# ShawnHymel/ei-keyword-spotting

Hardware: AMD Instinct MI355X
Metric: 1s@16kHz clips/sec (MFCC+CNN) (higher is better)
Workload: dtype f32

## Files before the change

### ei-keyword-spotting_amd/csrc/kws_device.h

```cpp
#pragma once
#include <hip/hip_runtime.h>
#include <stdint.h>
#include <float.h>
#include <type_traits>

#include "kws_plan.h"
#include "../../include/kws/kws_synth.h"

#pragma clang fp contract(off)

#define KWS_WAVE 64

__device__ __forceinline__ int sel_count(const int *sel, int n_clips) { return sel ? min(sel[0], n_clips) : n_clips; }
__device__ __forceinline__ int sel_clip(const int *sel, int i) { return sel ? sel[1 + i] : i; }

#define WAVE_SYNC()                                                   \
    do {                                                              \
        __builtin_amdgcn_fence(__ATOMIC_RELEASE, "wavefront");        \
        __builtin_amdgcn_wave_barrier();                              \
        __builtin_amdgcn_fence(__ATOMIC_ACQUIRE, "wavefront");        \
    } while (0)

__device__ __forceinline__ int ring_out_row(const KwsDspPlan &P, int r) { return P.ring_rows ? (P.ring_row0 + r) % P.ring_rows : r; }
__device__ __forceinline__ int ring_in_row(const KwsDspPlan &P, int i) { return (P.ring_rows && i < P.ring_rows) ? (i + P.ring_head) % P.ring_rows : i; }
// ... 11 lines not shown
__device__ __forceinline__ cf cadd(cf a, cf b) { cf c; c.r = a.r + b.r; c.i = a.i + b.i; return c; }
__device__ __forceinline__ cf csub(cf a, cf b) { cf c; c.r = a.r - b.r; c.i = a.i - b.i; return c; }

__device__ __forceinline__ void bfly4(cf &f0, cf &f1, cf &f2, cf &f3, cf t1, cf t2, cf t3)
{
    cf s0 = cmul(f1, t1), s1 = cmul(f2, t2), s2 = cmul(f3, t3);
    cf s5 = csub(f0, s1);
    f0 = cadd(f0, s1);
    cf s3 = cadd(s0, s2), s4 = csub(s0, s2);
    f2 = csub(f0, s3);
    f0 = cadd(f0, s3);
    f1.r = s5.r + s4.i;
    f1.i = s5.i - s4.r;
    f3.r = s5.r - s4.i;
    f3.i = s5.i + s4.r;
}

__device__ __forceinline__ void bfly4_unit(cf &f0, cf &f1, cf &f2, cf &f3)
{
    const cf s0 = f1, s1 = f2, s2 = f3;
    cf s5 = csub(f0, s1);
    f0 = cadd(f0, s1);
    cf s3 = cadd(s0, s2), s4 = csub(s0, s2);
    f2 = csub(f0, s3);
    f0 = cadd(f0, s3);
    f1.r = s5.r + s4.i;
    f1.i = s5.i - s4.r;
    f3.r = s5.r - s4.i;
    f3.i = s5.i + s4.r;
}

typedef int fast_i2 __attribute__((ext_vector_type(2), aligned(4)));

__device__ __forceinline__ cf exact_point(fast_i2 v, float pre_cof)
{
    const float prev = (float)(v.x >> 16) * (1.0f / 32768.0f);
    const float lo = (float)(short)(v.y & 0xffff) * (1.0f / 32768.0f);
    const float hi = (float)(v.y >> 16) * (1.0f / 32768.0f);
    cf z;
    const float pl = pre_cof * prev;
    z.r = lo - pl;
    const float ph_ = pre_cof * lo;
    z.i = hi - ph_;
    return z;
}

// ... 164 lines not shown
```

### ei-keyword-spotting_amd/csrc/kws_fast.h

```cpp
#pragma once
#include <stdint.h>

#include "kws_plan.h"

#define KWS_FAST_MAX_BLOCKS 8
#define KWS_FAST_NZ_MAX 12
#define KWS_FAST_NZ2 8
#define KWS_FAST_DCT_GROUPS 5
#define KWS_FAST_MEL_CHUNK 8
#define KWS_FAST_CMVN_EXT 8
#define KWS_FAST_XS 144
#define KWS_FAST_WAVE 64
#ifndef KWS_FAST_WPS
#define KWS_FAST_WPS 2
#endif
#define KWS_FAST_ZF 320

struct KwsFastBlock {
    int in_w, in_c, in_cp;
    int out_c, taps, pad_left, out_w;
    int pool, pool_stride, pool_w;
    int in_stride;
    int m_tiles, n_tiles;
    int vrows;
// ... 35 lines not shown
    int guard_off;
    int guard_cep_off;
    float v_net_feat;
    float g_c1, g_c2, v_net, lvl_inv;
    float c0_factor, c0_abs, c0_rel, c0_inv_rows;
    int pad_off;
    int sil_off;
    float sys_t2;
    int fs, f_floats, r1_floats, wave_floats, shared_floats, n_waves;
    int zero_off;
    int sink_off;
    int stash_off;
    const float *shared_init;
    int qnet, q_floats;
    int mfe;
    int fuse, n_blocks;
    KwsFastBlock blk[KWS_FAST_MAX_BLOCKS];
    int fc_in, fc_out, fc_w_off, fc_b_off;
    float fc_min, fc_max, beta;
    int n_labels;
    int wps;
    int twl_off;
    int *tickets;
};
```

### ei-keyword-spotting_amd/csrc/kws_fast.hip

```cpp
#include <atomic>

#include "kws_device.h"
#include "kws_fast.h"
#if KWS_FAST_WPS >= 3
#define kws_fast_kernel kws_fast_kernel_w3
#define kws_launch_fast kws_launch_fast_w3
#define kws_launch_fast_prof kws_launch_fast_prof_w3
#endif
#include "kws_nn_int8_dev.h"

typedef float v4f __attribute__((ext_vector_type(4)));
#if KWS_FAST_WPS >= 3
#define KWS_OPAQUE3(v) asm volatile("" : "+v"(v))
#define KWS_FAST_SINK (shared + FP.sink_off)
#else
#define KWS_OPAQUE3(v) do { } while (0)
#define KWS_FAST_SINK (F + FP.sink_off)
#endif
static_assert(KWS_FAST_ZF == KWS_ZF && KWS_FAST_WAVE == KWS_WAVE, "kws_fast.h mirrors kws_device.h");

template <int CTRL> __device__ __forceinline__ float dpp_mov(float v)
{
    return __int_as_float(__builtin_amdgcn_update_dpp(0, __float_as_int(v), CTRL, 0xf, 0xf, true));
}
// ... 222 lines not shown
        __builtin_amdgcn_sched_barrier(0);
        if (it + 1 >= n_it) break;
        const int tap1 = d1.y;
        d1 = steps[it + 3];
        fetch(d2, a0, b0);
        d0 = d2;
        __builtin_amdgcn_sched_barrier(0);
        clip_rows(tap1, a1);
        mfmas(a1, b1);
        __builtin_amdgcn_sched_barrier(0);
    }
    __builtin_amdgcn_s_setprio(0);
    if (t_loop) *t_loop = clock64();
    fast_conv_finish<MT, NT>(k, acc, vout, stage, sstride, shared, lane, sink, 1.0f);
    return 1.0f;
}

typedef _Float16 v8h __attribute__((ext_vector_type(8)));
typedef _Float16 v2h __attribute__((ext_vector_type(2)));
typedef const __attribute__((address_space(1))) char *kws_gptr;
typedef const __attribute__((address_space(1))) v8h *kws_gv8h;
#define KWS_FAST_HP 16

template <int T>
__device__ __forceinline__ float fast_split_trips(float *__restrict__ img, int items, int in_c, int in_cp, int in_stride, int lane, unsigned inv, int ppr)
{
    float2 v[T];
    int off[T];
    int pc[T];
#pragma unroll
    for (int u = 0; u < T; ++u) {
        const int i = min(lane + KWS_WAVE * u, items - 1);
        const int r = (int)(__umul24((unsigned)i, inv) >> 20), p2 = 2 * (i - __mul24(r, ppr));
        const int ro = __mul24(r, in_stride);
        v[u] = *(const float2 *)(img + ro + p2);
        off[u] = 4 * ro + 2 * p2;
        pc[u] = p2;
    }
#pragma unroll
    for (int u = 0; u < T; ++u) asm volatile("" : "+v"(v[u].x), "+v"(v[u].y));
    float mx = 0.0f;
#pragma unroll
    for (int u = 0; u < T; ++u) {
        v[u].x = pc[u] < in_c ? v[u].x : 0.0f;
        v[u].y = pc[u] + 1 < in_c ? v[u].y : 0.0f;
        mx = fmaxf(mx, fmaxf(fabsf(v[u].x), fabsf(v[u].y)));
    }
    mx = wave_max(mx);
    const int e = __builtin_amdgcn_readfirstlane(min(max(__builtin_amdgcn_frexp_expf(mx), -100), 100));
    const float s = ldexpf(1.0f, 14 - e);
    WAVE_SYNC();
    char *const ib = (char *)img;
    const int lo_off = 2 * in_cp;
#pragma unroll
    for (int u = 0; u < T; ++u) {
        const float y0 = v[u].x * s, y1 = v[u].y * s;
        const _Float16 h0 = (_Float16)y0, h1 = (_Float16)y1;
        const float d0 = y0 - (float)h0, d1 = y1 - (float)h1;
        const v2h hi = { h0, h1 }, lo = { (_Float16)d0, (_Float16)d1 };
        *(v2h *)(ib + off[u]) = hi;
        *(v2h *)(ib + off[u] + lo_off) = lo;
    }
    WAVE_SYNC();
    return ldexpf(1.0f, e - 14);
}

__device__ __forceinline__ float fast_split_image(float *__restrict__ img, int in_w, int in_c, int in_cp, int in_stride, int lane, unsigned ppr_inv20)
{
    const int ppr = in_cp >> 1, items = in_w * ppr;
    if (items <= 4 * KWS_WAVE) return fast_split_trips<4>(img, items, in_c, in_cp, in_stride, lane, ppr_inv20, ppr);
    if (items <= 8 * KWS_WAVE) return fast_split_trips<8>(img, items, in_c, in_cp, in_stride, lane, ppr_inv20, ppr);
    return fast_split_trips<KWS_FAST_HP>(img, items, in_c, in_cp, in_stride, lane, ppr_inv20, ppr);
}

template <int MT>
__device__ __forceinline__ float fast_conv_small_h(const KwsFastBlock &k, float *__restrict__ in, float *__restrict__ stage, int sstride,
                                                   const float *__restrict__ shared, int zero_off, int lane, float *__restrict__ sink)
{
    constexpr int KSM = 8;
    const int lm = lane & 15, lq = lane >> 4, n_ks = k.h_ks;
    const kws_gptr bg = (kws_gptr)k.h_b_global + lane * 16;
    v8h bh[KSM], blo[KSM];
#pragma unroll
    for (int ks = 0; ks < KSM; ++ks) {
        const int kc = min(ks, n_ks - 1);
        bh[ks] = *(kws_gv8h)(bg + (kc * 2) * (KWS_WAVE * 16));
        blo[ks] = *(kws_gv8h)(bg + (kc * 2 + 1) * (KWS_WAVE * 16));
    }
    const float inv_s = fast_split_image(in, k.in_w, k.in_c, k.in_cp, k.in_stride, lane, k.inv_ppr20);
    v4f acc[MT][1];
#pragma unroll
    for (int mt = 0; mt < MT; ++mt) acc[mt][0] = v4f{ 0.f, 0.f, 0.f, 0.f };
    const int rowb = k.in_stride * 4, in_w = k.in_w, lo_off = 2 * k.in_cp;
    const int row0 = lm - k.pad_left;
    const char *const abase = (const char *)in + row0 * rowb;
// ... 484 lines not shown
    if constexpr (QCP != 0) {
        unsigned char *const qs = (unsigned char *)(lds + FP.shared_floats);
        const KwsNnPlan &QN = *QNp;
        for (int i = threadIdx.x * 4; i < QN.blk[0].out_c * 256; i += blockDim.x * 4) *(int *)(qs + i) = *(const int *)(QN.blk[0].add_lut + i);
        for (int i = threadIdx.x * 4; i < QN.blk[1].out_c * 256; i += blockDim.x * 4) *(int *)(qs + 32 * 256 + i) = *(const int *)(QN.blk[1].add_lut + i);
        (void)nn_head_stage(QN, qs + Q_HEAD);
        nn_mfma_stage_lds<QCP == 0 ? 16 : QCP>(QN, (v4i *)(qs + Q_WB1), (v4i *)(qs + Q_WB2), (int *)(qs + Q_RQ));
    }
    if constexpr (FROM_CEP)
        for (int i = lane; i < FP.wave_floats; i += KWS_WAVE) F[i] = 0.0f;
    __syncthreads();

    const int nfr = P.n_frames, ncep = P.n_cepstral, NF = 8 * DG;
    const int n_tail = (nfr >= KWS_FAST_MEL_CHUNK && (nfr & 7) != 0 && (nfr & 7) <= 2) ? (nfr & 7) : 0;
    const int n_pass = n_tail ? nfr / KWS_FAST_MEL_CHUNK : (nfr + KWS_FAST_MEL_CHUNK - 1) / KWS_FAST_MEL_CHUNK;
    const int fs = FP.fs;
    float *img = F;
    float *elog = F + nfr * fs;
    constexpr int NZ2 = DG > 4 ? KWS_FAST_NZ2 : 1;
    const float *dct_frag = shared + FP.dct_off;
    const int pstride = FP.pstride;
    const int n_waves = blockDim.x >> 6;
    const float pre_cof = P.pre_cof, pscale = P.inv_fft * (1.0f / 1073741824.0f) * 0.25f;
    const int frame_stride = P.frame_stride, n_samples = P.n_samples;
    const float *cnt_tab = shared + FP.cnt_off;
    const int *upd_tab = (const int *)(shared + FP.upd_off);
    const float *ext_tab = FP.ext_off >= 0 ? shared + FP.ext_off : nullptr;
    const float inv_win = FP.inv_win;
    const float *guard_tab = shared + (FROM_CEP ? FP.guard_cep_off : FP.guard_off);
    const int *pad_idx = (const int *)(shared + FP.pad_off);
    const int win_size = P.win_size, prow = nfr + 2 * P.pad;
    const int cr = FP.cr, n_blocks = FP.n_blocks, n_labels = FP.n_labels;
    long long ph[KWS_FAST_NPHASE] = { 0 }, tlast = PROF ? clock64() : 0;

    const int clip_stride = gridDim.x * n_waves;
    float *const stash = F + FP.stash_off;
    bool have_stash = false;
    const int n_sel = FROM_CEP ? sel_count(sel, n_clips) : n_clips;
#if KWS_FAST_WPS >= 3
    int *const tk = FP.tickets;
    int tv = 0;
    int ni = 0;
    auto draw = [&]() { if (ni < n_sel && lane == 0) tv = __hip_atomic_fetch_add(tk, 1, __ATOMIC_RELAXED, __HIP_MEMORY_SCOPE_AGENT); };
    draw();
    ni = clip_stride + __builtin_amdgcn_readfirstlane(tv);
    draw();
    for (int ci = blockIdx.x * n_waves + wave; ci < n_sel; ci = ni, ni = ni < n_sel ? clip_stride + __builtin_amdgcn_readfirstlane(tv) : ni, draw()) {
        const int clip = FROM_CEP ? sel_clip(sel, ci) : ci;
        const int next_ci = ni;
        const int next_clip = ni < n_sel ? ni : -1;
#else
    for (int ci = blockIdx.x * n_waves + wave; ci < n_sel; ci += clip_stride) {
        const int clip = FROM_CEP ? sel_clip(sel, ci) : ci;
        const int next_ci = ci + clip_stride;
        const int next_clip = ci + clip_stride < n_sel ? ci + clip_stride : -1;
#endif
        int lane_c = lane;
        asm volatile("" : "+v"(lane_c));
        const int fl = lane_c & 7, fg = lane_c >> 3;
        const int nbA = (fl >> 2) + 4 * (fl & 3);
        const cf a1 = to_cf(P.tw[16]), a2 = to_cf(P.tw[32]), a3 = to_cf(P.tw[48]);
        const cf b1 = to_cf(P.tw[4 * fl]), b2 = to_cf(P.tw[8 * fl]), b3 = to_cf(P.tw[12 * fl]);
#if KWS_FAST_WPS >= 3
        const float *const twl_c = shared + FP.twl_off + 24 * fl, *const twl_s = shared + FP.twl_off + 192 + 16 * fl;
#else
        cf c1[4], c2[4], c3[4];
    #pragma unroll
        for (int a = 0; a < 4; ++a) { c1[a] = to_cf(P.tw[fl + 8 * a]); c2[a] = to_cf(P.tw[2 * (fl + 8 * a)]); c3[a] = to_cf(P.tw[3 * (fl + 8 * a)]); }
        cf stw[8];
    #pragma unroll
        for (int q = 0; q < 8; ++q) {
            const int k = fl + 8 * (q & 3) + 32 * (q >> 2);
            stw[q] = to_cf(P.stw[(k == 0 ? KWS_NC / 2 : k) - 1]);
        }
#endif
        const int xwr = fg * KWS_FAST_XS + 18 * fl;
        const int xrd = fg * KWS_FAST_XS + 2 * fl;
        const int partner = (lane_c & ~7) | ((8 - fl) & 7);
        const int half = lane_c >> 5, t = lane_c & 31;
        const int start1 = FP.tap_start1[lane_c], start2 = FP.tap_start2[lane_c];
        float lvl_sum = 0.0f;
        float w1[NZ], w2[NZ2];
    #pragma unroll
        for (int n = 0; n < NZ; ++n) w1[n] = FP.tap_w1[lane_c * KWS_FAST_NZ_MAX + n];
// ... 59 lines not shown
                if (s2 >= 2 * pairs) break;
                float xv[2][NZ];
#pragma unroll
                for (int s = 0; s < 2; ++s)
#pragma unroll
                    for (int n = 0; n < NZ; ++n) xv[s][n] = p1[(s2 + s) * pstride + n];
#pragma unroll
                for (int s = 0; s < 2; ++s) {
                    float acc = 0.0f;
#pragma unroll
                    for (int n = 0; n < NZ; ++n) acc = __fmaf_rn(xv[s][n], w1[n], acc);
                    macc[s2 + s] = acc;
                }
            }
            float acc2 = 0.0f;
            if (DG > 4) {
                float xv2[NZ2];
#pragma unroll
                for (int n = 0; n < NZ2; ++n) xv2[n] = p2[n];
#pragma unroll
                for (int n = 0; n < NZ2; ++n) acc2 = __fmaf_rn(xv2[n], w2[n], acc2);
            }
            macc[4] = acc2;
#pragma unroll
            for (int s = 0; s < 5; ++s) {
                const float a = macc[s] == 0.0f ? FLT_EPSILON : macc[s];
                macc[s] = MFE ? a : fast_log(a);
            }
#pragma unroll
            for (int s = 0; s < 4; ++s) {
                const int slot = 4 * half + s;
                if (slot < nfc && t < NF) img[(fbase + slot) * fs + t + (slot == 1 ? adj1 : 0)] = macc[s];
            }
            if (DG > 4 && sl2 < nfc && j2 < NF) img[(fbase + sl2) * fs + j2 + (sl2 == 1 ? adj1 : 0)] = macc[4];
        };
        fast_i2 nxt[2][8];
        fetch(0, nxt);
        int touched = touch(1);
        const bool pair_tail = n_tail == 1 && !have_stash && next_clip >= 0;
        int touched_tail = 0;
        const int16_t *const xnext = pcm + (size_t)max(next_clip, 0) * n_samples;
        if (pair_tail && lane_c < 8) touched_tail = *(const int *)(xnext + (nfr - 1) * frame_stride + 32 * lane_c);
        for (int q = 0; q < n_pass; ++q) {
            const int fbase = KWS_FAST_MEL_CHUNK * q;
            const int f = fbase + fg;
            const bool live = f < nfr;
            cf u[4][4];
            {
                cf z[2][8];
#pragma unroll
                for (int blk = 0; blk < 2; ++blk)
#pragma unroll
                    for (int i = 0; i < 8; ++i) z[blk][i] = fast_point(nxt[blk][i], pre_cof);
                if (f == 0 && fl == 0) {
                    fast_i2 v = nxt[0][0];
                    v.y = v.x;
                    v.x = wrap_prev << 16;
                    z[0][0] = fast_point(v, pre_cof);
                }
                fetch(q + 1, nxt);
                asm volatile("" : : "v"(touched));
                touched = touch(q + 2);
                FPH(0);
#pragma unroll
                for (int blk = 0; blk < 2; ++blk) {
                    cf sm[4], df[4];
#pragma unroll
                    for (int i = 0; i < 4; ++i) { sm[i] = cadd(z[blk][2 * i], z[blk][2 * i + 1]); df[i] = csub(z[blk][2 * i], z[blk][2 * i + 1]); }
                    bfly4_unit(sm[0], sm[1], sm[2], sm[3]);
                    bfly4(df[0], df[1], df[2], df[3], a1, a2, a3);
#pragma unroll
                    for (int i = 0; i < 4; ++i) { z[blk][2 * i] = sm[i]; z[blk][2 * i + 1] = df[i]; }
                }
#pragma unroll
                for (int rnd = 0; rnd < 2; ++rnd) {
#pragma unroll
                    for (int r = 0; r < 8; ++r) *(float2 *)(xw + xwr + 2 * r) = make_float2(z[rnd][r].r, z[rnd][r].i);
                    WAVE_SYNC();
#pragma unroll
                    for (int b = 0; b < 2; ++b)
#pragma unroll
                        for (int a = 0; a < 4; ++a) {
                            const float2 v = *(const float2 *)(xw + xrd + 18 * a + 72 * b);
                            u[a][2 * rnd + b].r = v.x; u[a][2 * rnd + b].i = v.y;
                        }
                    WAVE_SYNC();
                }
            }
#pragma unroll
            for (int b = 0; b < 4; ++b) bfly4(u[0][b], u[1][b], u[2][b], u[3][b], b1, b2, b3);
#pragma unroll
#if KWS_FAST_WPS >= 3
            for (int a = 0; a < 4; ++a) {
// ... 19 lines not shown
                float esum = 0.0f;
#pragma unroll
                for (int qq = 0; qq < 8; ++qq) {
                    const int a = qq & 3, b = qq >> 2;
                    cf other;
                    other.r = __int_as_float(__builtin_amdgcn_ds_bpermute(partner << 2, __float_as_int(u[3 - a][3 - b].r)));
                    other.i = __int_as_float(__builtin_amdgcn_ds_bpermute(partner << 2, __float_as_int(u[3 - a][3 - b].i)));
                    cf fpk = u[a][b];
                    int k = fl + 8 * a + 32 * b;
                    {
                        const int o = qq == 0 ? 8 : 16 - qq;
                        other.r = lane0 ? u[o & 3][o >> 2].r : other.r;
                        other.i = lane0 ? u[o & 3][o >> 2].i : other.i;
                        if (qq == 0) { fpk.r = lane0 ? u[0][2].r : fpk.r; fpk.i = lane0 ? u[0][2].i : fpk.i; k = lane0 ? KWS_NC / 2 : k; }
                    }
                    cf fpnk; fpnk.r = other.r; fpnk.i = -other.i;
                    const cf f1k = cadd(fpk, fpnk), f2k = csub(fpk, fpnk);
                    const cf twv = cmul(f2k, stw[qq]);
                    cf lo, hi;
                    lo.r = f1k.r + twv.r;
                    lo.i = f1k.i + twv.i;
                    hi.r = f1k.r - twv.r;
                    hi.i = twv.i - f1k.i;
                    const float plo = __fmaf_rn(lo.r, lo.r, lo.i * lo.i) * pscale;
                    const float phi = __fmaf_rn(hi.r, hi.r, hi.i * hi.i) * pscale;
                    prow[k] = plo;
                    esum += (qq == 0 && lane0) ? 0.0f : plo;
                    esum += phi;
                    prow[KWS_NC - k] = phi;
                }
                if (fl == 0) {
                    const float dc = u[0][0].r + u[0][0].i, ny = u[0][0].r - u[0][0].i;
#if KWS_FAST_WPS >= 3
                    const float pdc = ((dc * dc) * pscale) * 4.0f, pny = ((ny * ny) * pscale) * 4.0f;
#else
                    const float pdc = (dc * dc) * (4.0f * pscale), pny = (ny * ny) * (4.0f * pscale);
#endif
                    esum += pdc + pny;
                    prow[0] = pdc;
                }
                esum = oct_sum(esum);
                if (fl == 0 && live) elog[f] = fast_log(esum == 0.0f ? FLT_EPSILON : esum);
            }
            FPH(2);

            mel_phase(fbase, min(KWS_FAST_MEL_CHUNK, nfr - fbase), 2, 0);
            WAVE_SYNC();
            FPH(3);
        }

        asm volatile("" : : "v"(touched_tail));
        if (n_tail == 1 && have_stash) {
            if (lane_c < NF) img[(nfr - 1) * fs + lane_c] = stash[lane_c];
            if (lane_c == 47) elog[nfr - 1] = stash[47];
            have_stash = false;
            WAVE_SYNC();
        } else if (n_tail) {
            const int16_t *const xb_t = (pair_tail && half == 1) ? xnext : xbase;
            const int ft = pair_tail ? nfr - 1 : KWS_FAST_MEL_CHUNK * n_pass + half;
            const bool live_t = ft < nfr;
            const int s0 = min(ft, nfr - 1) * frame_stride + 8 * t;
            const int4 rawv = *(const int4 *)(xb_t + s0);
            const int rawp = s0 == 0 ? wrap_prev : (int)xb_t[s0 - 1];
            const int k01 = t & 1, g01 = t >> 1, n0 = (g01 >> 2) + 4 * (g01 & 3), K2 = t & 7, G2 = t >> 3;
// ... 47 lines not shown
                const cf st1 = to_cf(P.stw[t]), st2 = to_cf(P.stw[t + 32]);
                cf fpk[2], fq[2];
#pragma unroll
                for (int rep = 0; rep < 2; ++rep) {
                    const int k = t + 1 + 32 * rep;
                    fpk[rep] = ld_cf(zb, k);
                    fq[rep] = ld_cf(zb, KWS_NC - k);
                }
                const float2 d0 = *(const float2 *)zb;
                float *prow = pw + half * pstride;
                float esum = 0.0f;
#pragma unroll
                for (int rep = 0; rep < 2; ++rep) {
                    const int k = t + 1 + 32 * rep;
                    const cf stw_ = rep ? st2 : st1;
                    cf fpnk; fpnk.r = fq[rep].r; fpnk.i = -fq[rep].i;
                    const cf f1k = cadd(fpk[rep], fpnk), f2k = csub(fpk[rep], fpnk);
                    const cf twv = cmul(f2k, stw_);
                    cf lo, hi;
                    lo.r = f1k.r + twv.r;
                    lo.i = f1k.i + twv.i;
                    hi.r = f1k.r - twv.r;
                    hi.i = twv.i - f1k.i;
                    const float plo = __fmaf_rn(lo.r, lo.r, lo.i * lo.i) * pscale;
                    const float phi = __fmaf_rn(hi.r, hi.r, hi.i * hi.i) * pscale;
                    if (k != KWS_NC / 2) {
                        esum += plo;
                        prow[k] = plo;
                    }
                    esum += phi;
                    prow[KWS_NC - k] = phi;
                }
                if (t == 0) {
                    const float dc = d0.x + d0.y, ny = d0.x - d0.y;
                    const float pdc = (dc * dc) * (4.0f * pscale), pny = (ny * ny) * (4.0f * pscale);
                    esum += pdc + pny;
                    prow[0] = pdc;
                }
                esum = half_wave_sum(esum);
                if (t == 0 && live_t) *((pair_tail && half == 1) ? stash + 47 : elog + ft) = fast_log(esum == 0.0f ? FLT_EPSILON : esum);
            }
            mel_phase(KWS_FAST_MEL_CHUNK * n_pass, pair_tail ? 2 : n_tail, 1, pair_tail ? (int)(stash - img) - nfr * fs : 0);
            have_stash = pair_tail;
            WAVE_SYNC();
        }

        if constexpr (!MFE) {
            int lane_l = lane;
            asm volatile("" : "+v"(lane_l));
            const int lm = lane_l & 15, lq = lane_l >> 4;
            float dB[DG][2][2];
#pragma unroll
            for (int g = 0; g < DG; ++g)
#pragma unroll
                for (int i = 0; i < 2; ++i)
#pragma unroll
                    for (int nt = 0; nt < 2; ++nt) dB[g][i][nt] = dct_frag[((g * 2 + i) * 2 + nt) * KWS_WAVE + lane_l];
            const float *arow = img + lm * fs + 2 * lq;
            float e0 = 0.0f;
            if (lane_l < nfr) e0 = elog[lane_l];
            v4f acc[4][2];
            __builtin_amdgcn_s_setprio(1);
// ... 405 lines not shown
```

### ei-keyword-spotting_amd/csrc/kws_fast_plan.cpp

```cpp
#include "kws_internal.h"
#include <atomic>
#include <cstdlib>

static const int kLdsBytes = 160 * 1024;

static int round_up(int v, int m) { return (v + m - 1) / m * m; }

static uint16_t f32_to_f16(float f)
{
    uint32_t u;
    memcpy(&u, &f, sizeof u);
    const uint32_t sign = (u >> 16) & 0x8000u;
    u &= 0x7fffffffu;
    if (u >= 0x47800000u) return (uint16_t)(sign | (u > 0x7f800000u ? 0x7e00u : 0x7c00u));
    if (u < 0x38800000u) {
        if (u < 0x33000000u) return (uint16_t)sign;
        const int shift = 126 - (int)(u >> 23);
        const uint32_t m = (u & 0x7fffffu) | 0x800000u;
        uint32_t h = m >> shift;
        const uint32_t rem = m & ((1u << shift) - 1u), half = 1u << (shift - 1);
        if (rem > half || (rem == half && (h & 1u))) h++;
        return (uint16_t)(sign | h);
    }
    uint32_t h = ((u - 0x38000000u) >> 13);
// ... 32 lines not shown
{
    h->fast_sil_row.clear();
    if (h->model.dsp.block == DSP_BLOCK_MFE || h->dsp.generic) return;
    const int nfr = h->dsp.n_frames, ncep = h->dsp.n_cepstral;
    const size_t ns = (size_t)h->dsp.n_samples, nv = (size_t)nfr * (size_t)ncep;
    int16_t *d_pcm = nullptr;
    float *d_cep = nullptr;
    std::vector<float> cep(nv, 0.0f);
    bool ok = hipMalloc((void **)&d_pcm, ns * sizeof(int16_t) + 64) == hipSuccess && hipMalloc((void **)&d_cep, nv * sizeof(float)) == hipSuccess;
    ok = ok && hipMemset(d_pcm, 0, ns * sizeof(int16_t) + 64) == hipSuccess && hipMemset(d_cep, 0xff, nv * sizeof(float)) == hipSuccess;
    ok = ok && spectral_device(h, h->dsp, d_pcm, 0, 1, d_cep, nullptr, nullptr) == EI_IMPULSE_OK && hipDeviceSynchronize() == hipSuccess;
    ok = ok && hipMemcpy(cep.data(), d_cep, nv * sizeof(float), hipMemcpyDeviceToHost) == hipSuccess;
    if (d_pcm) (void)hipFree(d_pcm);
    if (d_cep) (void)hipFree(d_cep);
    (void)hipGetLastError();
    if (!ok) return;
    for (int c = 0; c < ncep; c++) {
        if (!std::isfinite(cep[(size_t)c])) return;
        for (int r = 1; r < nfr; r++)
            if (memcmp(&cep[(size_t)r * ncep + c], &cep[(size_t)c], sizeof(float)) != 0) return;
    }
    if (fabsf(cep[0] - logf(FLT_EPSILON)) > 1.0e-3f) return;
    h->fast_sil_row.assign(cep.begin(), cep.begin() + ncep);
}

static void build_guard(kws_handle *h, KwsFastPlan &F, std::vector<float> &shared)
{
    const int ncep = h->dsp.n_cepstral, NF = h->model.dsp.num_filters, nfr = h->dsp.n_frames;
    const bool refit = h->is_float && h->gain.calibrated;
    float a0 = refit ? kAlpha0 : 1.0e-7f, ad = refit ? -1.0f : kAlphaDct, as = refit ? kAlphaStale : 4.0e-8f, kappa = refit ? kKappa : 0.5e-6f, scale = 1.0f;
    const float e0 = refit ? kAbs0 : 6.0e-7f, kappa_s = refit ? kKappaStale : 0.35e-6f, kappa_0 = refit ? kKappa0 : 0.5e-6f;
    if (const char *ev = KWS_DEV_ENV("KWS_DEV_FAST_GUARD_SCALE")) { scale = (float)atof(ev); h->fast_dev_overrides |= 1; }
    if (const char *ev = KWS_DEV_ENV("KWS_DEV_FAST_GUARD")) { (void)sscanf(ev, "%f,%f,%f,%f", &a0, &ad, &as, &kappa); h->fast_dev_overrides |= 2; }
    if (KWS_DEV_ENV("KWS_DEV_FAST_NO_RERUN")) h->fast_dev_overrides |= 4;
#ifdef KWS_DEV_SWITCHES
    if (h->fast_dev_overrides) {
        static std::atomic<bool> said{ false };
        if (!said.exchange(true))
            fprintf(stderr, "libkws_mi355x: a KWS_DEV_FAST_* development switch is set: KWS_MODE_FAST results are OUTSIDE the documented tolerance\n");
    }
#endif
    std::vector<float> gain((size_t)ncep, 0.0f);
    if (h->is_float && h->gain.calibrated) gain = h->gain.col;
    else for (float &g : gain) g = 4.0f / (kGuardLin * sqrtf((float)(nfr * ncep)));
    h->fast_gain_used = gain;
    F.g_c1 = (kGuardK * kGuardLin / kGuardScoreTol) * (kGuardK * kGuardLin / kGuardScoreTol);
// ... 24 lines not shown
                coef[1] = 0.0f;
                coef[2] = g * kap;
                coef[3] = c == 0 ? 0.0f : g * kKappaSilent;
            }
            for (int k = 0; k < 4; k++) {
                shared.push_back(coef[k]);
                if (c < ncep) h->fast_guard_coef[tier][k].push_back(k == 1 ? coef[k] * unit : coef[k]);
            }
        }
    }
    {
        int entry = 3;
        for (int tier = 1; tier >= 0; tier--) {
            double v = (double)F.v_net;
            for (int c = 0; c < ncep; c++) {
                const double dev = c == 0 ? 1.5 : c <= NF / 2 ? 1.0 : 0.5, mean = c == 0 ? 8.0 : c <= NF / 2 ? 1.0 : 2.2;
                const double b = ((double)h->fast_guard_coef[tier][0][(size_t)c] + (double)h->fast_guard_coef[tier][1][(size_t)c] * 10.0 +
                                  (double)h->fast_guard_coef[tier][2][(size_t)c] * mean) / dev;
                v += (double)nfr * b * b;
            }
            if (v * (double)std::max(F.g_c1 / 16.0f, F.g_c2) <= 1.0) entry = tier + 1;
        }
        if (const char *ev = KWS_DEV_ENV("KWS_DEV_FAST_ENTRY")) entry = std::max(1, std::min(3, atoi(ev)));
        h->fast_entry_tier = entry;
    }
    std::vector<int> pmap;
    h_pad_map(h->dsp.n_frames, h->dsp.pad, pmap);
    {
        const int nfr = h->dsp.n_frames, win = h->model.dsp.win_size;
        int mult = win;
        for (int r = 0; r < nfr; r++) {
            std::vector<int> cnt((size_t)nfr, 0);
            for (int p = r; p < r + win; p++) cnt[(size_t)pmap[(size_t)p]]++;
            for (int v : cnt) mult = std::min(mult, v);
        }
        F.c0_factor = sqrtf((float)mult * (float)nfr / (float)win) * 0.98f;
        const float budget = 1.0f / std::max(F.g_c1 / 16.0f, F.g_c2);
        const float per_dev = gain[0] * sqrtf((float)nfr / (kC0Share * budget));
        F.c0_abs = scale * kFloorCep * per_dev;
        F.c0_rel = scale * std::min(kappa, kappa_0) * per_dev;
        F.c0_inv_rows = 1.0f / (float)nfr;
    }
    F.sys_t2 = (h->is_float && h->gain.calibrated) ? kSysRatio * kSysRatio : 0.0f;
    F.pad_off = (int)shared.size();
    for (int v : pmap) { float f; memcpy(&f, &v, sizeof f); shared.push_back(f); }
    F.sil_off = -1;
    if ((int)h->fast_sil_row.size() == ncep && !KWS_DEV_ENV("KWS_DEV_FAST_NO_SILENT_ROW")) {
        while (shared.size() & 3) shared.push_back(0.0f);
        F.sil_off = (int)shared.size();
        for (int c = 0; c < 32; c++) shared.push_back((c >= 1 && c <= NF / 2 && c < ncep) ? h->fast_sil_row[(size_t)c] : 0.0f);
    }
}

static EI_IMPULSE_ERROR build_fast_dsp(kws_handle *h, KwsFastPlan &F, std::vector<float> &shared)
{
    const Model &m = h->model;
    const DspCfg &c = m.dsp;
    const KwsDspPlan &P = h->dsp;
    const int NF = c.num_filters, nfr = P.n_frames, ncep = P.n_cepstral;
    F.mfe = c.block == DSP_BLOCK_MFE ? 1 : 0;
    if (P.generic) return fail(KWS_ERROR_UNSUPPORTED_MODEL, "fast mode serves the configurations of the tuned MFCC kernel (fft 256, 32 / 40 filters, "
                                                            "up to 52 aligned frames); this model runs on the general kernels");
    if (c.fft_length != 256) return fail(KWS_ERROR_UNSUPPORTED_MODEL, "fast mode: fft_length %d (kernel is built for 256)", c.fft_length);
    if (NF != 32 && NF != 40) return fail(KWS_ERROR_UNSUPPORTED_MODEL, "fast mode: %d mel filters (the kernel is instantiated for 32 and 40)", NF);
    if ((ncep <= 16 || F.wps >= 3) && nfr <= 52) { F.cr = 13; F.cg = 16; }
    else if (nfr <= 51) { F.cr = 17; F.cg = 20; }
    else return fail(KWS_ERROR_UNSUPPORTED_MODEL, "fast mode: %d frames x %d cepstra outside the cmvnw layouts", nfr, ncep);
    if (nfr < 2) return fail(KWS_ERROR_UNSUPPORTED_MODEL, "fast mode: %d frames", nfr);

    const uint32_t fs_hz = m.frequency;
    const uint32_t high = c.high_frequency == 0 ? fs_hz / 2 : (uint32_t)c.high_frequency;
    const std::vector<float> fb = h_filterbank(NF, P.n_bins, fs_hz, (uint32_t)c.low_frequency, high, c.quantize_fb != 0);
    int bmin = P.n_bins, bmax = -1, max_nz = 0;
    std::vector<std::vector<std::pair<int, float>>> taps(NF);
    for (int j = 0; j < NF; j++) {
        for (int k = 0; k < P.n_bins; k++) {
            const float w = fb[(size_t)k * NF + j];
            if (w != 0.0f) { taps[j].push_back({ k, w }); bmin = std::min(bmin, k); bmax = std::max(bmax, k); }
        }
        max_nz = std::max(max_nz, (int)taps[j].size());
    }
    if (bmax < 0) { bmin = 0; bmax = 0; }
    if (max_nz > KWS_FAST_NZ_MAX) return fail(KWS_ERROR_UNSUPPORTED_MODEL, "fast mode: mel filter with %d taps (at most %d)", max_nz, KWS_FAST_NZ_MAX);
    if (bmax > P.n_bins - 2) return fail(KWS_ERROR_UNSUPPORTED_MODEL, "fast mode: a mel filter reads the Nyquist bin");
    bmin = 0;
    bmax = P.n_bins - 2;
// ... 5 lines not shown
        for (size_t n = 1; n < taps[j].size(); n++)
            if (taps[j][n].first != taps[j][n - 1].first + 1) return fail(KWS_ERROR_UNSUPPORTED_MODEL, "fast mode: mel filter %d has a gap", j);
        (j < 32 ? nz1 : nz2) = std::max(j < 32 ? nz1 : nz2, (int)taps[j].size());
    }
    if (nz1 > KWS_FAST_NZ_MAX || nz2 > KWS_FAST_NZ2)
        return fail(KWS_ERROR_UNSUPPORTED_MODEL, "fast mode: mel filters with %d / %d taps (at most %d / %d)", nz1, nz2, KWS_FAST_NZ_MAX, KWS_FAST_NZ2);
    F.nz = nz1 <= 4 ? 4 : nz1 <= 8 ? 8 : KWS_FAST_NZ_MAX;
    F.pstride = (F.nbins + std::max(F.nz, KWS_FAST_NZ2)) | 1;
    if (F.pstride <= 136) F.pstride = 136;
    auto tap_table = [&](auto filter_of_lane, int width, std::vector<int> &start, std::vector<float> &w) {
        start.assign(KWS_FAST_WAVE, 0);
        w.assign((size_t)KWS_FAST_WAVE * width, 0.0f);
        for (int lane = 0; lane < KWS_FAST_WAVE; lane++) {
            const int j = filter_of_lane(lane);
            if (j < 0 || j >= NF || taps[j].empty()) continue;
            start[lane] = taps[j][0].first - bmin;
            for (size_t n = 0; n < taps[j].size(); n++) w[(size_t)lane * width + n] = taps[j][n].second;
        }
    };
    std::vector<int> s1, s2;
    std::vector<float> tw1, tw2;
    tap_table([&](int lane) { return lane & 31; }, KWS_FAST_NZ_MAX, s1, tw1);
    tap_table([&](int lane) { return F.nf2p ? 32 + (lane & (F.nf2p - 1)) : -1; }, KWS_FAST_NZ2, s2, tw2);

    F.dct_groups = NF / 8;
    F.dct_nt = (NF / 2 + 1 + 15) / 16;
    if (F.dct_nt > 2) return fail(KWS_ERROR_UNSUPPORTED_MODEL, "fast mode: DCT output tiles");
    F.dct_nt = 2;
    F.stale_scale = P.dct_s1;
    std::vector<float> frag((size_t)F.dct_groups * 2 * F.dct_nt * KWS_FAST_WAVE, 0.0f);
    for (int g = 0; g < F.dct_groups; g++)
        for (int i = 0; i < 2; i++)
            for (int nt = 0; nt < F.dct_nt; nt++)
                for (int lane = 0; lane < KWS_FAST_WAVE; lane++) {
                    const int k = 8 * g + 2 * (lane >> 4) + i, n = 16 * nt + (lane & 15);
                    double v = 0.0;
                    if (n <= NF / 2) v = 2.0 * cos(M_PI * (double)n * (double)(2 * k + 1) / (double)(2 * NF)) * (double)(n == 0 ? P.dct_s0 : P.dct_s1);
                    frag[(((size_t)g * 2 + i) * F.dct_nt + nt) * KWS_FAST_WAVE + lane] = (float)v;
                }

    std::vector<int> pmap;
    h_pad_map(nfr, P.pad, pmap);
    const int ng = KWS_FAST_WAVE / F.cg, win = c.win_size;
    F.inv_win = 1.0f / (float)win;
    build_guard(h, F, shared);
    while (shared.size() & 3) shared.push_back(0.0f);
// ... 339 lines not shown
```

### ei-keyword-spotting_amd/csrc/kws_internal.h

```cpp
#pragma once
#include <hip/hip_runtime.h>

#include <float.h>
#include <math.h>
#include <stdarg.h>
#include <stdio.h>
#include <stdlib.h>
#include <string.h>
#include <time.h>

#include <mutex>
#include <string>
#include <map>
#include <vector>

#include "../../include/kws/kws.h"
#include "kws_plan.h"
#include "kws_fast.h"

int kws_launch_spectral(const KwsDspPlan &P, const void *pcm, int pcm_is_float, int n_clips, float *mfcc_out, const float *wrap,
                        int out_stride, int grid_cap, hipStream_t stream, const int *sel = nullptr);
int kws_launch_maf(float *scores, float *running_sum, float *maf_buf, int n, int buf_idx, int taps, hipStream_t stream);
int kws_launch_unring(const float *src, float *dst, int n_streams, int rows, int cols, int ring_rows, int head, hipStream_t stream);
int kws_launch_mfe(const KwsDspPlan &P, const void *pcm, int pcm_is_float, int n_clips, float *mel_out, float *energy_out, const float *wrap,
// ... 77 lines not shown
enum { DSP_BLOCK_MFCC = 0, DSP_BLOCK_MFE = 1 };
struct DspCfg {
    int axes, num_cepstral, num_filters, fft_length, win_size, low_frequency, high_frequency, pre_shift;
    float frame_length, frame_stride, pre_cof;
    int block = DSP_BLOCK_MFCC;
    int quantize_fb = 0;
};
struct Model {
    std::vector<Tensor> t;
    std::vector<Node> n;
    std::vector<std::string> labels;
    uint32_t t_in = 0, t_out = 0, raw_sample_count = 0, frequency = 0, nn_input_frame_size = 0;
    DspCfg dsp;
};

bool parse_model(const void *blob, size_t nbytes, Model &m);
float h_fast_log(float a);
float h_freq_to_mel(float f);
float h_mel_to_freq(float mel);
void h_linspace(float start, float stop, uint32_t number, float *out);
std::vector<float> h_filterbank(int num_filter, int coefficients, uint32_t fs, uint32_t low, uint32_t high, bool quantize = false);
float h_quantize_zero_one(float value);
void h_twiddles(int nfft, std::vector<float2> &tw);
void h_super_twiddles(int ncfft, std::vector<float2> &st);
void h_pad_map(int rows, int pad, std::vector<int> &map);
int32_t h_srdhm(int32_t a, int32_t b);
int32_t h_rdivpot(int32_t x, int e);
void h_quantize_multiplier(double m, int32_t *q, int *shift);
int32_t h_wadd(int32_t a, int32_t b);
int32_t h_wsub(int32_t a, int32_t b);
int32_t h_sat_shl(int32_t x, int e);
int32_t h_exp_interval(int32_t a);
int32_t h_exp_neg_q5_26(int32_t a);
void h_act_range(int activation, float scale, int32_t zp, int32_t *amin, int32_t *amax);
int h_out_size(int padding, int image, int filter, int stride, int dil);
int h_pad_amount(int stride, int dil, int in_size, int filter, int out);

struct kws_handle {
    Model model;
    int device = 0;
    int n_cu = 256;
    KwsDspPlan dsp{};
    KwsNnPlan nn{};
    bool is_float = false;
    KwsNnPlanF32 nnf{};
    const KwsNnPlanF32 *d_nnf = nullptr;
// ... 156 lines not shown
```

Baseline: 52.61 million.

## Fold power scale into mel weights, specialize radix-4 twiddles, streamline split-image addressing

Specializes one radix-4 butterfly for the fixed twiddles (c,-c),(0,-1),(-c,-c), so it needs fewer multiplies. It moves the per-bin power scale out of the per-bin loops: the scale is folded into the mel filter weights when that is exact, or applied to the mel accumulators otherwise, and to the energy after the reduction. The fp16 split of the image now walks LDS addresses incrementally with explicit LDS pointers, and skips the padding masks when channels are not padded. Host checks confirm the twiddle pattern and that the fold is exact, so rounding stays bit-compatible, at the cost of extra plan complexity.

```diff
diff --git a/ei-keyword-spotting_amd/csrc/kws_device.h b/ei-keyword-spotting_amd/csrc/kws_device.h
--- a/ei-keyword-spotting_amd/csrc/kws_device.h
+++ b/ei-keyword-spotting_amd/csrc/kws_device.h
@@ -57,6 +57,31 @@
     cf s5 = csub(f0, s1);
     f0 = cadd(f0, s1);
     cf s3 = cadd(s0, s2), s4 = csub(s0, s2);
+    f2 = csub(f0, s3);
+    f0 = cadd(f0, s3);
+    f1.r = s5.r + s4.i;
+    f1.i = s5.i - s4.r;
+    f3.r = s5.r - s4.i;
+    f3.i = s5.i + s4.r;
+}
+
+__device__ __forceinline__ void bfly4_k1(cf &f0, cf &f1, cf &f2, cf &f3, float c, float e)
+{
+    const float p1 = f1.r * c, q1 = f1.i * c, p3 = f3.r * c, q3 = f3.i * c;
+    const float er = f2.r * e, ei = f2.i * e;
+    cf s0, s1;
+    s0.r = p1 + q1;
+    s0.i = q1 - p1;
+    s1.r = er + f2.i;
+    s1.i = ei - f2.r;
+    const float s2r = q3 - p3, n2 = p3 + q3;
+    cf s5 = csub(f0, s1);
+    f0 = cadd(f0, s1);
+    cf s3, s4;
+    s3.r = s0.r + s2r;
+    s3.i = s0.i - n2;
+    s4.r = s0.r - s2r;
+    s4.i = s0.i + n2;
     f2 = csub(f0, s3);
     f0 = cadd(f0, s3);
     f1.r = s5.r + s4.i;
diff --git a/ei-keyword-spotting_amd/csrc/kws_fast.h b/ei-keyword-spotting_amd/csrc/kws_fast.h
--- a/ei-keyword-spotting_amd/csrc/kws_fast.h
+++ b/ei-keyword-spotting_amd/csrc/kws_fast.h
@@ -81,4 +81,5 @@
     int wps;
     int twl_off;
     int *tickets;
+    int pfold;
 };
diff --git a/ei-keyword-spotting_amd/csrc/kws_fast.hip b/ei-keyword-spotting_amd/csrc/kws_fast.hip
--- a/ei-keyword-spotting_amd/csrc/kws_fast.hip
+++ b/ei-keyword-spotting_amd/csrc/kws_fast.hip
@@ -268,35 +268,54 @@
 typedef const __attribute__((address_space(1))) v8h *kws_gv8h;
 #define KWS_FAST_HP 16
 
-template <int T>
-__device__ __forceinline__ float fast_split_trips(float *__restrict__ img, int items, int in_c, int in_cp, int in_stride, int lane, unsigned inv, int ppr)
+typedef __attribute__((address_space(3))) char *kws_lptr;
+typedef float v2f __attribute__((ext_vector_type(2)));
+template <int T, bool PAD>
+__device__ __forceinline__ float fast_split_trips(float *__restrict__ img, int in_w, int in_c, int in_cp, int in_stride, int lane, unsigned inv, int ppr)
 {
     float2 v[T];
     int off[T];
-    int pc[T];
+    int pc[PAD ? T : 1];
+    constexpr int CLAMP_FROM = T > 4 ? T / 2 : 0;
+    const int base = (int)(unsigned)(uintptr_t)(kws_lptr)(char *)img;
+    const int rowb = 4 * in_stride, rowh = 4 * ppr;
+    const int qr = (int)(__umul24((unsigned)KWS_WAVE, inv) >> 20), qp = KWS_WAVE - __mul24(qr, ppr);
+    const int d_hb = 4 * qp, d_ra = __mul24(qr, rowb) + 2 * d_hb, carry_ra = rowb - 2 * rowh;
+    const int ra_last = base + __mul24(in_w - 1, rowb) + 2 * rowh - 8, off_last = ra_last - (rowh - 4);
+    const int r0 = (int)(__umul24((unsigned)lane, inv) >> 20);
+    int hb = 4 * (lane - __mul24(r0, ppr));
+    int ra = base + __mul24(r0, rowb) + 2 * hb;
 #pragma unroll
     for (int u = 0; u < T; ++u) {
-        const int i = min(lane + KWS_WAVE * u, items - 1);
-        const int r = (int)(__umul24((unsigned)i, inv) >> 20), p2 = 2 * (i - __mul24(r, ppr));
-        const int ro = __mul24(r, in_stride);
-        v[u] = *(const float2 *)(img + ro + p2);
-        off[u] = 4 * ro + 2 * p2;
-        pc[u] = p2;
+        int ru = ra, ou = ra - hb;
+        if (u >= CLAMP_FROM) { ru = min(ru, ra_last); ou = min(ou, off_last); }
+        const v2f rd = *(const __attribute__((address_space(3))) v2f *)(kws_lptr)(uintptr_t)(unsigned)ru;
+        v[u].x = rd.x; v[u].y = rd.y;
+        off[u] = ou;
+        if constexpr (PAD) pc[u] = (ru - ou) >> 1;
+        if (u + 1 < T) {
+            hb += d_hb;
+            ra += d_ra;
+            const bool carry = hb >= rowh;
+            hb = carry ? hb - rowh : hb;
+            ra = carry ? ra + carry_ra : ra;
+        }
     }
 #pragma unroll
     for (int u = 0; u < T; ++u) asm volatile("" : "+v"(v[u].x), "+v"(v[u].y));
     float mx = 0.0f;
 #pragma unroll
     for (int u = 0; u < T; ++u) {
-        v[u].x = pc[u] < in_c ? v[u].x : 0.0f;
-        v[u].y = pc[u] + 1 < in_c ? v[u].y : 0.0f;
+        if constexpr (PAD) {
+            v[u].x = pc[u] < in_c ? v[u].x : 0.0f;
+            v[u].y = pc[u] + 1 < in_c ? v[u].y : 0.0f;
+        }
         mx = fmaxf(mx, fmaxf(fabsf(v[u].x), fabsf(v[u].y)));
     }
     mx = wave_max(mx);
     const int e = __builtin_amdgcn_readfirstlane(min(max(__builtin_amdgcn_frexp_expf(mx), -100), 100));
     const float s = ldexpf(1.0f, 14 - e);
     WAVE_SYNC();
-    char *const ib = (char *)img;
     const int lo_off = 2 * in_cp;
 #pragma unroll
     for (int u = 0; u < T; ++u) {
@@ -304,8 +323,8 @@
         const _Float16 h0 = (_Float16)y0, h1 = (_Float16)y1;
         const float d0 = y0 - (float)h0, d1 = y1 - (float)h1;
         const v2h hi = { h0, h1 }, lo = { (_Float16)d0, (_Float16)d1 };
-        *(v2h *)(ib + off[u]) = hi;
-        *(v2h *)(ib + off[u] + lo_off) = lo;
+        *(__attribute__((address_space(3))) v2h *)(kws_lptr)(uintptr_t)(unsigned)off[u] = hi;
+        *(__attribute__((address_space(3))) v2h *)(kws_lptr)(uintptr_t)(unsigned)(off[u] + lo_off) = lo;
     }
     WAVE_SYNC();
     return ldexpf(1.0f, e - 14);
@@ -314,9 +333,14 @@
 __device__ __forceinline__ float fast_split_image(float *__restrict__ img, int in_w, int in_c, int in_cp, int in_stride, int lane, unsigned ppr_inv20)
 {
     const int ppr = in_cp >> 1, items = in_w * ppr;
-    if (items <= 4 * KWS_WAVE) return fast_split_trips<4>(img, items, in_c, in_cp, in_stride, lane, ppr_inv20, ppr);
-    if (items <= 8 * KWS_WAVE) return fast_split_trips<8>(img, items, in_c, in_cp, in_stride, lane, ppr_inv20, ppr);
-    return fast_split_trips<KWS_FAST_HP>(img, items, in_c, in_cp, in_stride, lane, ppr_inv20, ppr);
+    if (in_c == in_cp) {
+        if (items <= 4 * KWS_WAVE) return fast_split_trips<4, false>(img, in_w, in_c, in_cp, in_stride, lane, ppr_inv20, ppr);
+        if (items <= 8 * KWS_WAVE) return fast_split_trips<8, false>(img, in_w, in_c, in_cp, in_stride, lane, ppr_inv20, ppr);
+        return fast_split_trips<KWS_FAST_HP, false>(img, in_w, in_c, in_cp, in_stride, lane, ppr_inv20, ppr);
+    }
+    if (items <= 4 * KWS_WAVE) return fast_split_trips<4, true>(img, in_w, in_c, in_cp, in_stride, lane, ppr_inv20, ppr);
+    if (items <= 8 * KWS_WAVE) return fast_split_trips<8, true>(img, in_w, in_c, in_cp, in_stride, lane, ppr_inv20, ppr);
+    return fast_split_trips<KWS_FAST_HP, true>(img, in_w, in_c, in_cp, in_stride, lane, ppr_inv20, ppr);
 }
 
 template <int MT>
@@ -847,6 +871,7 @@
     const int pstride = FP.pstride;
     const int n_waves = blockDim.x >> 6;
     const float pre_cof = P.pre_cof, pscale = P.inv_fft * (1.0f / 1073741824.0f) * 0.25f;
+    const bool pfold = FP.pfold != 0;
     const int frame_stride = P.frame_stride, n_samples = P.n_samples;
     const float *cnt_tab = shared + FP.cnt_off;
     const int *upd_tab = (const int *)(shared + FP.upd_off);
@@ -884,7 +909,7 @@
         asm volatile("" : "+v"(lane_c));
         const int fl = lane_c & 7, fg = lane_c >> 3;
         const int nbA = (fl >> 2) + 4 * (fl & 3);
-        const cf a1 = to_cf(P.tw[16]), a2 = to_cf(P.tw[32]), a3 = to_cf(P.tw[48]);
+        const float a_c = P.tw[16].x, a_e = P.tw[32].x;
         const cf b1 = to_cf(P.tw[4 * fl]), b2 = to_cf(P.tw[8 * fl]), b3 = to_cf(P.tw[12 * fl]);
 #if KWS_FAST_WPS >= 3
         const float *const twl_c = shared + FP.twl_off + 24 * fl, *const twl_s = shared + FP.twl_off + 192 + 16 * fl;
@@ -990,6 +1015,10 @@
                 for (int n = 0; n < NZ2; ++n) acc2 = __fmaf_rn(xv2[n], w2[n], acc2);
             }
             macc[4] = acc2;
+            if (!pfold) {
+#pragma unroll
+                for (int s = 0; s < 5; ++s) macc[s] *= pscale;
+            }
 #pragma unroll
             for (int s = 0; s < 5; ++s) {
                 const float a = macc[s] == 0.0f ? FLT_EPSILON : macc[s];
@@ -1036,7 +1065,7 @@
 #pragma unroll
                     for (int i = 0; i < 4; ++i) { sm[i] = cadd(z[blk][2 * i], z[blk][2 * i + 1]); df[i] = csub(z[blk][2 * i], z[blk][2 * i + 1]); }
                     bfly4_unit(sm[0], sm[1], sm[2], sm[3]);
-                    bfly4(df[0], df[1], df[2], df[3], a1, a2, a3);
+                    bfly4_k1(df[0], df[1], df[2], df[3], a_c, a_e);
 #pragma unroll
                     for (int i = 0; i < 4; ++i) { z[blk][2 * i] = sm[i]; z[blk][2 * i + 1] = df[i]; }
                 }
@@ -1102,8 +1131,8 @@
                     lo.i = f1k.i + twv.i;
                     hi.r = f1k.r - twv.r;
                     hi.i = twv.i - f1k.i;
-                    const float plo = __fmaf_rn(lo.r, lo.r, lo.i * lo.i) * pscale;
-                    const float phi = __fmaf_rn(hi.r, hi.r, hi.i * hi.i) * pscale;
+                    const float plo = __fmaf_rn(lo.r, lo.r, lo.i * lo.i);
+                    const float phi = __fmaf_rn(hi.r, hi.r, hi.i * hi.i);
                     prow[k] = plo;
                     esum += (qq == 0 && lane0) ? 0.0f : plo;
                     esum += phi;
@@ -1111,15 +1140,11 @@
                 }
                 if (fl == 0) {
                     const float dc = u[0][0].r + u[0][0].i, ny = u[0][0].r - u[0][0].i;
-#if KWS_FAST_WPS >= 3
-                    const float pdc = ((dc * dc) * pscale) * 4.0f, pny = ((ny * ny) * pscale) * 4.0f;
-#else
-                    const float pdc = (dc * dc) * (4.0f * pscale), pny = (ny * ny) * (4.0f * pscale);
-#endif
+                    const float pdc = (dc * dc) * 4.0f, pny = (ny * ny) * 4.0f;
                     esum += pdc + pny;
                     prow[0] = pdc;
                 }
-                esum = oct_sum(esum);
+                esum = oct_sum(esum) * pscale;
                 if (fl == 0 && live) elog[f] = fast_log(esum == 0.0f ? FLT_EPSILON : esum);
             }
             FPH(2);
@@ -1213,8 +1238,8 @@
                     lo.i = f1k.i + twv.i;
                     hi.r = f1k.r - twv.r;
                     hi.i = twv.i - f1k.i;
-                    const float plo = __fmaf_rn(lo.r, lo.r, lo.i * lo.i) * pscale;
-                    const float phi = __fmaf_rn(hi.r, hi.r, hi.i * hi.i) * pscale;
+                    const float plo = __fmaf_rn(lo.r, lo.r, lo.i * lo.i);
+                    const float phi = __fmaf_rn(hi.r, hi.r, hi.i * hi.i);
                     if (k != KWS_NC / 2) {
                         esum += plo;
                         prow[k] = plo;
@@ -1224,11 +1249,11 @@
                 }
                 if (t == 0) {
                     const float dc = d0.x + d0.y, ny = d0.x - d0.y;
-                    const float pdc = (dc * dc) * (4.0f * pscale), pny = (ny * ny) * (4.0f * pscale);
+                    const float pdc = (dc * dc) * 4.0f, pny = (ny * ny) * 4.0f;
                     esum += pdc + pny;
                     prow[0] = pdc;
                 }
-                esum = half_wave_sum(esum);
+                esum = half_wave_sum(esum) * pscale;
                 if (t == 0 && live_t) *((pair_tail && half == 1) ? stash + 47 : elog + ft) = fast_log(esum == 0.0f ? FLT_EPSILON : esum);
             }
             mel_phase(KWS_FAST_MEL_CHUNK * n_pass, pair_tail ? 2 : n_tail, 1, pair_tail ? (int)(stash - img) - nfr * fs : 0);
diff --git a/ei-keyword-spotting_amd/csrc/kws_fast_plan.cpp b/ei-keyword-spotting_amd/csrc/kws_fast_plan.cpp
--- a/ei-keyword-spotting_amd/csrc/kws_fast_plan.cpp
+++ b/ei-keyword-spotting_amd/csrc/kws_fast_plan.cpp
@@ -78,6 +78,17 @@
     }
     if (fabsf(cep[0] - logf(FLT_EPSILON)) > 1.0e-3f) return;
     h->fast_sil_row.assign(cep.begin(), cep.begin() + ncep);
+}
+
+bool fast_k1_twiddles(int ncfft)
+{
+    std::vector<float2> tw;
+    h_twiddles(ncfft, tw);
+    if (ncfft < 8 || (ncfft & 7) != 0 || (int)tw.size() < 3 * (ncfft / 8) + 1) return false;
+    auto bits = [](float f) { uint32_t u; memcpy(&u, &f, sizeof u); return u; };
+    const float2 t1 = tw[(size_t)ncfft / 8], t2 = tw[(size_t)ncfft / 4], t3 = tw[(size_t)3 * (ncfft / 8)];
+    const float c = t1.x;
+    return c > 0.0f && bits(t1.y) == bits(-c) && bits(t3.x) == bits(-c) && bits(t3.y) == bits(-c) && bits(t2.y) == bits(-1.0f);
 }
 
 static void build_guard(kws_handle *h, KwsFastPlan &F, std::vector<float> &shared)
@@ -148,6 +159,7 @@
             if (v * (double)std::max(F.g_c1 / 16.0f, F.g_c2) <= 1.0) entry = tier + 1;
         }
         if (const char *ev = KWS_DEV_ENV("KWS_DEV_FAST_ENTRY")) entry = std::max(1, std::min(3, atoi(ev)));
+        if (!fast_k1_twiddles(h->model.dsp.fft_length / 2)) entry = std::max(entry, 2);
         h->fast_entry_tier = entry;
     }
     std::vector<int> pmap;
@@ -188,6 +200,7 @@
     if (P.generic) return fail(KWS_ERROR_UNSUPPORTED_MODEL, "fast mode serves the configurations of the tuned MFCC kernel (fft 256, 32 / 40 filters, "
                                                             "up to 52 aligned frames); this model runs on the general kernels");
     if (c.fft_length != 256) return fail(KWS_ERROR_UNSUPPORTED_MODEL, "fast mode: fft_length %d (kernel is built for 256)", c.fft_length);
+    if (F.mfe && !fast_k1_twiddles(c.fft_length / 2)) return fail(KWS_ERROR_UNSUPPORTED_MODEL, "fast mode: the transform's twiddles are not the ones the kernel is written for");
     if (NF != 32 && NF != 40) return fail(KWS_ERROR_UNSUPPORTED_MODEL, "fast mode: %d mel filters (the kernel is instantiated for 32 and 40)", NF);
     if ((ncep <= 16 || F.wps >= 3) && nfr <= 52) { F.cr = 13; F.cg = 16; }
     else if (nfr <= 51) { F.cr = 17; F.cg = 20; }
@@ -239,6 +252,17 @@
     std::vector<float> tw1, tw2;
     tap_table([&](int lane) { return lane & 31; }, KWS_FAST_NZ_MAX, s1, tw1);
     tap_table([&](int lane) { return F.nf2p ? 32 + (lane & (F.nf2p - 1)) : -1; }, KWS_FAST_NZ2, s2, tw2);
+
+    {
+        const float ps = P.inv_fft * (1.0f / 1073741824.0f) * 0.25f;
+        int ex = 0;
+        bool fold = ps >= FLT_MIN && frexpf(ps, &ex) == 0.5f;
+        for (const std::vector<float> *t : { &tw1, &tw2 })
+            for (float w : *t)
+                if (w != 0.0f && !(fabsf(w * ps) >= FLT_MIN && std::isfinite(w))) fold = false;
+        F.pfold = fold ? 1 : 0;
+        if (fold) { for (float &w : tw1) w *= ps; for (float &w : tw2) w *= ps; }
+    }
 
     F.dct_groups = NF / 8;
     F.dct_nt = (NF / 2 + 1 + 15) / 16;
diff --git a/ei-keyword-spotting_amd/csrc/kws_internal.h b/ei-keyword-spotting_amd/csrc/kws_internal.h
--- a/ei-keyword-spotting_amd/csrc/kws_internal.h
+++ b/ei-keyword-spotting_amd/csrc/kws_internal.h
@@ -123,6 +123,7 @@
 std::vector<float> h_filterbank(int num_filter, int coefficients, uint32_t fs, uint32_t low, uint32_t high, bool quantize = false);
 float h_quantize_zero_one(float value);
 void h_twiddles(int nfft, std::vector<float2> &tw);
+bool fast_k1_twiddles(int ncfft);
 void h_super_twiddles(int ncfft, std::vector<float2> &st);
 void h_pad_map(int rows, int pad, std::vector<int> &map);
 int32_t h_srdhm(int32_t a, int32_t b);
```

New measurement: 51.78 million. -1.6%, worse.
